# wenbowen123/BundleTrack

Hardware: AMD Instinct MI355X
Metric: Gauss-Newton iters/sec (K=15, 2k corr/frame-pair) + achieved HBM GB/s (higher is better)
Workload: dtype f32

## Files before the change

bundletrack_amd/csrc/btba_api.hip:

```cpp
#include <chrono>

#include "btba_host_common.hpp"
#include "btba_kernels.hpp"
#include "btba_solve_general.hpp"
#include "btba_chain.hpp"
#include "btba_solve_small.hpp"
#include "btba_solve_mid.hpp"

thread_local int btba_host::g_last_hip_error = 0;

extern "C" {

void btba_params_default(btba_params *p)
{
    if (!p) return;
    p->n_gn_iters = 7;
    p->n_pcg_iters = 5;
    p->robust_delta = 0.005f;
    p->dense_dist_thresh = 0.02f;
    p->dense_normal_thresh = (float)std::cos(45.0 / 180.0 * M_PI);
    p->depth_min = 0.1f;
    p->depth_max = 9999.0f;
    p->weight_sparse = 1.0f;
    p->weight_dense_depth = 1.0f;
// ... 541 lines not shown
        HIP_TRY(hipMemsetAsync(ws->dense_part.p, 0, sizeof(float) * (size_t)B * (Pd > 0 ? Pd : 1) * kDenseVals, ws->stream));
    }
    const bool compaction = use_zn && use_dense && (prm->flags & BTBA_FLAG_COMPACTION);
    const int chain_lay = zn_layout == 1 ? (compaction ? 3 : 1) : 0;
    const bool chain = chain_lay != 0 && !ws->chain_failed && ws->n_cus == 256 && ws->tune.chain > 0 && use_sparse && use_dense && !wsi && !wdi
                       && !trace && !atomic_sums && !a_global && !D.pre_assembled && N <= kChainMaxFrames && chunks <= kChainMaxParts && tiles <= kChainMaxParts
                       && !(prm->flags & (BTBA_FLAG_NO_FUSE | BTBA_FLAG_OVERLAP)) && !Z.frame_slot
                       && sizeof(float) * SolveLayout(N, D.n_dense_pairs, true, true).total <= kChainLdsBytes;
    const bool relayout = ws->tune.relayout && use_sparse && !corr24 && !pair_lens && !chain && prm->n_gn_iters >= 3 && !atomic_sums && !compaction
                          && (size_t)B * (size_t)corr_stride * sizeof(btba_entryj) >= ((size_t)4 << 20);
    if (relayout) { if ((rc = ws->corr24_tmp.ensure(sizeof(float2) * 192 * (((size_t)B * (size_t)corr_stride + 63) / 64)))) return rc; }
    const long long frames_bytes = use_dense ? (long long)B * N * npix * (use_zn ? 16 : 32) : 0;
    const long long corr_bytes = use_sparse ? (long long)B * (long long)corr_stride * (corr24 ? 24 : 32) : 0;
    const long long corr_per_instance = corr_bytes / B;
    int corr_nt_auto = B;
    if (use_dense && use_sparse && !compaction && frames_bytes + corr_bytes > ws->tune.last_level_cache)
        corr_nt_auto = (frames_bytes >= ws->tune.last_level_cache || corr_per_instance <= 0) ? 0 : (int)std::min<long long>(B, (ws->tune.last_level_cache - frames_bytes) / corr_per_instance);
    if (ws->tune.corr_nt_partial == 0 && corr_nt_auto < B) corr_nt_auto = 0;
    const int corr_nt_from = ws->tune.corr_nt >= 0 ? (ws->tune.corr_nt ? 0 : B) : corr_nt_auto;
    ChainDims Cn{};
    int plain_pairsum_in_lds = 0;
    auto pad32 = [](size_t floats) { return (floats + 31) & ~(size_t)31; };
    if (chain) {
        const int n_it = prm->n_gn_iters;
        D.pose_stride = (int)pad32(16 * (size_t)N); D.x_stride = (int)pad32(6 * (size_t)N);
        D.sp_stride = (unsigned)pad32((size_t)P * chunks * kSparseVals); D.dp_stride = (unsigned)pad32((size_t)Pd * tiles * kDenseVals);
        D.publish = 1;
        D.corr_nt_from = corr_nt_from;
        plain_pairsum_in_lds = D.pairsum_in_lds;
        D.pairsum_in_lds = 0;
        Cn.last_solve_external = 1;
        Cn.n_iter = n_it; Cn.n_inst = B; Cn.inst_per_xcd = (unsigned)((B + 7) / 8);
        Cn.items_d = (unsigned)tiles * (unsigned)D.n_dense_pairs; Cn.items_s = (unsigned)chunks * (unsigned)P;
        Cn.sparse_period = (unsigned)ws->tune.chain_sparse_period;
        if (Cn.sparse_period >= 2u && Cn.sparse_period * Cn.items_s > Cn.items_d + Cn.items_s) Cn.sparse_period = (Cn.items_d + Cn.items_s) / Cn.items_s;
        if (Cn.sparse_period < 2u) Cn.sparse_period = 0u;
        Cn.group = (Cn.sparse_period == 0u && ws->tune.chain_group > 1 && Cn.inst_per_xcd % (unsigned)ws->tune.chain_group == 0u && B % 8 == 0) ? (unsigned)ws->tune.chain_group : 1u;
        Cn.timeout_ticks = (long long)ws->tune.chain_timeout_ms * 100000ll;
        Cn.solve_prio = ws->tune.chain_solve_prio;
        Cn.debug_skip = ws->tune.chain_debug_skip;
        if (Cn.debug_skip & 16) D.publish = 0;
        Cn.pose_ring = (size_t)B * D.pose_stride; Cn.x_ring = (size_t)B * D.x_stride;
        Cn.sp_ring = (size_t)B * (size_t)D.sp_stride; Cn.dp_ring = (size_t)B * (size_t)D.dp_stride;
        Cn.ps_size = pad32((size_t)D.n_dense_pairs * kDenseVals); Cn.A_size = pad32((n + 2) * ld);
        if ((rc = ws->x.ensure(sizeof(float) * (n_it + 1) * Cn.x_ring))) return rc;
        if ((rc = ws->T.ensure(sizeof(float) * (n_it + 1) * Cn.pose_ring))) return rc;
        if ((rc = ws->Tinv.ensure(sizeof(float) * (n_it + 1) * Cn.pose_ring))) return rc;
        if ((rc = ws->sparse_part.ensure(sizeof(float) * n_it * Cn.sp_ring))) return rc;
        if ((rc = ws->dense_part.ensure(sizeof(float) * n_it * Cn.dp_ring))) return rc;
        if ((rc = ws->pairsum.ensure(sizeof(float) * (size_t)n_it * B * Cn.ps_size))) return rc;
        if ((rc = ws->big_A.ensure(sizeof(float) * (size_t)n_it * B * Cn.A_size))) return rc;
        const size_t sync_head = ((size_t)B * (n_it + 1) + 15) & ~(size_t)15;
        const size_t sync_ints = sync_head + (size_t)16 * B * (n_it + 1);
        if ((rc = ws->chain_sync.ensure(sizeof(int) * sync_ints))) return rc;
        if (!ws->chain_error) {
            HIP_TRY(hipHostMalloc(reinterpret_cast<void **>(&ws->chain_error), 64, hipHostMallocDefault));
            *ws->chain_error = 0;
        }
        HIP_TRY(hipMemsetAsync(ws->chain_sync.p, 0, sizeof(int) * sync_ints, ws->stream));
        Cn.flags = ws->chain_sync.as<int>(); Cn.arrivals = Cn.flags + B; Cn.published = Cn.flags + sync_head; Cn.error = ws->chain_error;
    }
    {
        const int total = B * N;
        if (chain) k_prepare_strided<<<(total + 63) / 64, 64, 0, ws->stream>>>(total, N, D.pose_stride, D.x_stride, poses, ws->x.as<float>(), ws->T.as<float>(), ws->Tinv.as<float>());
        else k_prepare<<<(total + 63) / 64, 64, 0, ws->stream>>>(total, poses, ws->x.as<float>(), ws->T.as<float>(), ws->Tinv.as<float>(), ws->tune.prepare_keep_T);
    }
    const uint32_t *lists_base = Z.lists;
    const int *counts_base = Z.counts;
    if (compaction && !lists_base) {
        if ((rc = ws->valid_lists.ensure(sizeof(uint32_t) * (size_t)B * N * npix))) return rc;
        if ((rc = ws->valid_counts.ensure(sizeof(int) * (size_t)B * N))) return rc;
        k_valid_lists<<<B * N, 1024, 0, ws->stream>>>(npix, reinterpret_cast<const float4 *>(Z.zn), ws->valid_lists.as<uint32_t>(), ws->valid_counts.as<int>(), nullptr);
        lists_base = ws->valid_lists.as<uint32_t>();
        counts_base = ws->valid_counts.as<int>();
    }
    if (Z.frame_slot && B != 1) return BTBA_EINVAL;
    D.frame_slot = Z.frame_slot;
    size_t blist_bytes = 0;
    if (!(zn_layout == 1 && use_dense && !compaction)) D.walk_blocks = 0;
    D.sparse_tail_256 = ws->tune.sparse_tail_256 >= 0 ? ws->tune.sparse_tail_256 : ((use_dense && !compaction) ? 256 : 0);
    if (D.walk_blocks) {
        const int bw = Wd / 8, bh = Hd / 8;
        const size_t band_blocks = (size_t)((bh + tiles - 1) / tiles) * bw;
        if (band_blocks > 1024) D.walk_blocks = 0;
        else {
            blist_bytes = 32 + sizeof(uint32_t) * band_blocks;
            if (ws->tune.block_skip) {
                if (Z.block_ranges) D.block_ranges = reinterpret_cast<const float2 *>(Z.block_ranges);
                else if (!Z.frame_slot) {
                    if ((rc = ws->block_ranges.ensure(sizeof(float2) * (size_t)B * N * bw * bh))) return rc;
                    k_block_ranges<<<dim3((unsigned)((bw * bh + kBlock / 64 - 1) / (kBlock / 64)), (unsigned)(B * N)), kBlock, 0, ws->stream>>>(Wd, Hd, reinterpret_cast<const float4 *>(Z.zn), nullptr, ws->block_ranges.as<float2>());
                    D.block_ranges = ws->block_ranges.as<float2>();
                }
            }
        }
    }
    int n_halves = (B >= 8 && (prm->flags & BTBA_FLAG_OVERLAP)) ? 2 : 1;
    if (n_halves == 2) n_halves = std::max(1, std::min({ ws->tune.overlap_groups, (int)btba_workspace::kMaxGroups, B / 2 }));
    for (int g = 1; g < n_halves; g++) {
        if (ws->aux_streams[g - 1]) continue;
        int prio_least = 0, prio_greatest = 0;
        HIP_TRY(hipDeviceGetStreamPriorityRange(&prio_least, &prio_greatest));
        HIP_TRY(hipStreamCreateWithPriority(&ws->aux_streams[g - 1], hipStreamNonBlocking, ws->tune.overlap_equal_prio ? 0 : prio_least));
        HIP_TRY(hipEventCreateWithFlags(&ws->ev_join[g - 1], hipEventDisableTiming));
        if (!ws->ev_fork) HIP_TRY(hipEventCreateWithFlags(&ws->ev_fork, hipEventDisableTiming));
    }
    struct Half { int b0, nb; hipStream_t st; } halves[btba_workspace::kMaxGroups];
    for (int g = 0; g < n_halves; g++) {
        const int lo = (int)((long long)B * g / n_halves), hi = (int)((long long)B * (g + 1) / n_halves);
        halves[g] = { lo, hi - lo, g == 0 ? ws->stream : ws->aux_streams[g - 1] };
    }
    if (n_halves > 1) {
        HIP_TRY(hipEventRecord(ws->ev_fork, ws->stream));
        for (int g = 1; g < n_halves; g++) HIP_TRY(hipStreamWaitEvent(ws->aux_streams[g - 1], ws->ev_fork, 0));
    }
    const size_t pairsum_floats = lds_pairs / sizeof(float);
    S.chain_iterations = 0;
    const size_t lut_bytes = sizeof(float) * (size_t)((Wd + Hd + 3) & ~3) + (zn_layout == 1 ? sizeof(float4) * (size_t)(Wd + Hd) : 0) + blist_bytes + (size_t)ws->tune.debug_lds_pad;
    if (chain) {
        const size_t chain_lds = std::max(lut_bytes, sizeof(float) * SolveLayout(N, D.n_dense_pairs, true, true).total);
        const unsigned per_inst = Cn.items_d + Cn.items_s + 1u;
        const unsigned grid = 8u * (unsigned)prm->n_gn_iters * Cn.inst_per_xcd * per_inst;
        if (!ws->tune.chain_trace_file.empty()) {
            const size_t trace_bytes = 32 * (size_t)grid + 64 * (size_t)prm->n_gn_iters * B;
            if ((rc = ws->chain_trace.ensure(trace_bytes))) return rc;
            HIP_TRY(hipMemsetAsync(ws->chain_trace.p, 0, trace_bytes, ws->stream));
            Cn.trace = ws->chain_trace.as<unsigned long long>();
            Cn.stamps = Cn.trace + 4 * (size_t)grid;
        }
        const float4 *corr_c = reinterpret_cast<const float4 *>(corr);
        size_t slot;
        if (Cn.debug_skip & 32) {
            ChainDims C1 = Cn;
            C1.n_iter = 1; C1.debug_skip |= 8; C1.trace = nullptr; C1.stamps = nullptr;
            const unsigned grid1 = 8u * Cn.inst_per_xcd * per_inst;
            if ((rc = ws->pairsum.ensure(sizeof(float) * (size_t)B * ((size_t)P * kSparseVals + (size_t)D.n_dense_pairs * kDenseVals + 64)))) return rc;
            for (int it = 0; it < prm->n_gn_iters; it++) {
                if ((rc = time_begin(ws, timing, 0, &slot))) return rc;
#define BTBA_CHAIN_ARGS1 D, C1, reinterpret_cast<const float4 *>(Z.zn), ws->T.as<float>(), ws->Tinv.as<float>(), ws->x.as<float>(), ws->dense_part.as<float>(), corr_c, pair_offsets, \
                        ws->sparse_part.as<float>(), compaction ? lists_base : nullptr, compaction ? counts_base : nullptr, ws->dense_pairs.as<int2>(), d_adj_off, d_adj, ws->solve_tab.as<int>(), \
                        ws->pairsum.as<float>(), ws->big_A.as<float>(), poses
                if (chain_lay == 1) k_chain<1><<<dim3(grid1), kBlock, chain_lds, ws->stream>>>(BTBA_CHAIN_ARGS1);
                else k_chain<3><<<dim3(grid1), kBlock, chain_lds, ws->stream>>>(BTBA_CHAIN_ARGS1);
#undef BTBA_CHAIN_ARGS1
                if ((rc = time_end(ws, slot))) return rc;
                if ((rc = time_begin(ws, timing, 2, &slot))) return rc;
                k_system_solve<false, false><<<B, kSolveBlock, lds_core, ws->stream>>>(D, it, ws->sparse_part.as<float>(), ws->dense_part.as<float>(), ws->dense_pairs.as<int2>(), d_adj_off, d_adj,
                    ws->x.as<float>(), ws->T.as<float>(), ws->Tinv.as<float>(), ws->pairsum.as<float>(), nullptr, nullptr, it == prm->n_gn_iters - 1 ? poses : nullptr, ws->solve_tab.as<int>());
                if ((rc = time_end(ws, slot))) return rc;
            }
            S.fused_sweeps = 1;
        } else {
        if ((rc = time_begin(ws, timing, 0, &slot))) return rc;
#define BTBA_CHAIN_ARGS D, Cn, reinterpret_cast<const float4 *>(Z.zn), ws->T.as<float>(), ws->Tinv.as<float>(), ws->x.as<float>(), ws->dense_part.as<float>(), corr_c, pair_offsets, \
                        ws->sparse_part.as<float>(), compaction ? lists_base : nullptr, compaction ? counts_base : nullptr, ws->dense_pairs.as<int2>(), d_adj_off, d_adj, ws->solve_tab.as<int>(), \
                        ws->pairsum.as<float>(), ws->big_A.as<float>(), poses
        if (chain_lay == 1) k_chain<1><<<dim3(grid), kBlock, chain_lds, ws->stream>>>(BTBA_CHAIN_ARGS);
        else k_chain<3><<<dim3(grid), kBlock, chain_lds, ws->stream>>>(BTBA_CHAIN_ARGS);
#undef BTBA_CHAIN_ARGS
        if ((rc = time_end(ws, slot))) return rc;
        if (Cn.last_solve_external) {
            const int il = prm->n_gn_iters - 1;
            SolveDims Dl = D;
            Dl.pairsum_in_lds = plain_pairsum_in_lds; Dl.publish = 0;
            if (!Dl.pairsum_in_lds) { if ((rc = ws->pairsum.ensure(std::max(sizeof(float) * (size_t)prm->n_gn_iters * B * Cn.ps_size, (size_t)B * lds_pairs + 16)))) return rc; }
            if ((rc = time_begin(ws, timing, 2, &slot))) return rc;
#define BTBA_LAST_SOLVE(LP) k_system_solve<LP, false><<<B, kSolveBlock, lds_bytes, ws->stream>>>(Dl, il, ws->sparse_part.as<float>() + il * Cn.sp_ring, ws->dense_part.as<float>() + il * Cn.dp_ring, \
                ws->dense_pairs.as<int2>(), d_adj_off, d_adj, ws->x.as<float>() + il * Cn.x_ring, ws->T.as<float>() + il * Cn.pose_ring, ws->Tinv.as<float>() + il * Cn.pose_ring, \
                ws->pairsum.as<float>(), nullptr, nullptr, poses, ws->solve_tab.as<int>())
// ... 798 lines not shown
```

bundletrack_amd/csrc/btba_kernels.hpp:

```cpp
#pragma once
#ifndef BTBA_FUSED_WAVES
#define BTBA_FUSED_WAVES 6
#endif
#if defined(BTBA_REFERENCE_ORDER) && !defined(BTBA_EXACT_DIV)
#define BTBA_EXACT_DIV 1
#endif
#include <type_traits>
#include <hip/hip_runtime.h>
#include <stdint.h>
#include "btba_device.hpp"

namespace btba {

constexpr int kBlock = 256;
constexpr int kSolveBlock = 1024;
constexpr int kSparseVals = 44;
constexpr int kDenseVals = 28;
constexpr float kEps = 0.000001f;
constexpr int kRedFloats = 4 * kSparseVals + 8;


struct SolveDims {
    int n_frames;
    int n_pairs;
    int n_dense_pairs;
    int npix, width, height;
    int sparse_chunks;
    int dense_tiles;
    int n_pcg;
    int use_sparse, use_dense;
    float fx, fy, cx, cy;
    float robust_delta, dist_thresh, normal_thresh, depth_min, depth_max;
    float dist2_thresh;
    float wm1, hm1, wm2, hm2;
    float w_sparse, w_dense;
    int64_t corr_stride;
    int trace_on;
    int64_t trace_record;
    int64_t tr_x, tr_T, tr_rhs, tr_prec, tr_pcg, tr_delta, tr_dpair, tr_A, tr_clk;
    int n_gn;
    int pairsum_in_lds;
    int pre_assembled;
    int walk_blocks;
    const int4 *dense_work;
    int work_formula;
    const float2 *block_ranges;
    int sparse_tail_256;
    int tile_major;
    int *order_flag;
    int atomic_sums;
    int corr24;
    int64_t corr_entry0;
    const uint32_t *pair_lens;
    float zn_ki[16];
    float zn_scale_w, zn_scale_h;
    int zn_simple;
    const int *frame_slot;
    int pose_stride, x_stride;
    unsigned sp_stride, dp_stride;
    float2 *corr24_out;
    unsigned long long *live_blocks;
    int publish;
    int corr_nt_from;
};

__device__ __forceinline__ size_t frame_slot_of(const SolveDims &D, size_t f) { return D.frame_slot ? (size_t)D.frame_slot[f] : f; }

__device__ __forceinline__ int pair_index(int i, int j, int n) { return i * n - i * (i + 1) / 2 + (j - i - 1); }

__device__ __forceinline__ Mat4 load_mat4(const float *p)
{
    Mat4 m;
    const float4 *q = reinterpret_cast<const float4 *>(p);
    float4 a = q[0], b = q[1], c = q[2], d = q[3];
    m.m[0] = a.x; m.m[1] = a.y; m.m[2] = a.z; m.m[3] = a.w;
    m.m[4] = b.x; m.m[5] = b.y; m.m[6] = b.z; m.m[7] = b.w;
    m.m[8] = c.x; m.m[9] = c.y; m.m[10] = c.z; m.m[11] = c.w;
    m.m[12] = d.x; m.m[13] = d.y; m.m[14] = d.z; m.m[15] = d.w;
    return m;
}
__device__ __forceinline__ Mat4 load_mat4_uniform(const float *p)
{
    Mat4 m;
    const float4 a = ld_const_f4(p), b = ld_const_f4(p + 4), c = ld_const_f4(p + 8), d = ld_const_f4(p + 12);
    m.m[0] = a.x; m.m[1] = a.y; m.m[2] = a.z; m.m[3] = a.w;
    m.m[4] = b.x; m.m[5] = b.y; m.m[6] = b.z; m.m[7] = b.w;
    m.m[8] = c.x; m.m[9] = c.y; m.m[10] = c.z; m.m[11] = c.w;
    m.m[12] = d.x; m.m[13] = d.y; m.m[14] = d.z; m.m[15] = d.w;
    return m;
}
__device__ __forceinline__ void store_mat4(float *p, const Mat4 &m)
{
    float4 *q = reinterpret_cast<float4 *>(p);
// ... 642 lines not shown
    const unsigned pb = (unsigned)b * (unsigned)D.pose_stride;
    dense_stage_M(red, T + pb + 16 * fi);
    DenseCtx C;
    C.Tij = mat_mul(load_mat4(Tinv + pb + 16 * fi), load_mat4(T + pb + 16 * fj));
#pragma unroll
    for (int e = 0; e < 12; e++) C.Tij.m[e] = __builtin_bit_cast(float, __builtin_amdgcn_readfirstlane(__builtin_bit_cast(int, C.Tij.m[e])));
    C.cam_t = nullptr; C.nrm_t = nullptr;
    C.fx = D.fx; C.fy = D.fy; C.cx = D.cx; C.cy = D.cy; C.depth_min = D.depth_min; C.depth_max = D.depth_max;
    C.normal_thresh = D.normal_thresh; C.dist2_thresh = D.dist_thresh * D.dist_thresh;
    C.delta = D.robust_delta; C.delta2 = D.robust_delta * D.robust_delta; C.w_dense = D.w_dense;
    C.W = D.width; C.H = D.height;
    const size_t slot_t = (size_t)__builtin_amdgcn_readfirstlane((int)frame_slot_of(D, fb + fi));
    const size_t slot_s = (size_t)__builtin_amdgcn_readfirstlane((int)frame_slot_of(D, fb + fj));
    const float4 *zn_t = zn + slot_t * (size_t)D.npix, *zn_s = zn + slot_s * (size_t)D.npix;
    const int n_src = LISTS ? valid_counts[slot_s] : D.npix;
    const uint32_t *list = LISTS ? valid_lists + slot_s * (size_t)D.npix : nullptr;
    const int per = (n_src + D.dense_tiles - 1) / D.dense_tiles;
    const int lo = min(n_src, per * tile), hi = min(n_src, per * (tile + 1));
    const float inv_w = 1.0f / (float)D.width;
    float acc[kDenseVals];
#pragma unroll
    for (int k = 0; k < kDenseVals; k++) acc[k] = 0.0f;

    int t = lo + (int)threadIdx.x;
    int s_n = (t < hi) ? (LISTS ? (int)list[t] : t) : 0;
    int px_i = s_n % D.width, py_i = s_n / D.width;
    const int step_x = kBlock % D.width, step_y = kBlock / D.width;
    float4 zs_n = make_float4(0.f, 0.f, 0.f, 0.f);
    if (t < hi) zs_n = zn_s[s_n];
    for (; t < hi; t += kBlock) {
        const float4 zs = zs_n;
        const int s = s_n;
        if (t + kBlock < hi) { s_n = LISTS ? (int)list[t + kBlock] : t + kBlock; zs_n = zn_s[s_n]; }
        int px, py;
        if (!LISTS) {
            px = px_i; py = py_i;
            px_i += step_x; py_i += step_y;
            if (px_i >= D.width) { px_i -= D.width; py_i++; }
        } else {
            py = (int)((float)s * inv_w);
            py -= (py * D.width > s) ? 1 : 0;
            py += ((py + 1) * D.width <= s) ? 1 : 0;
            px = s - py * D.width;
        }
        const float3 cp = zn_backproject<SIMPLE>(D.zn_ki, lut_x[px], lut_y[py], zs.x);
        const PixelGeom g = pixel_geom(C, make_float4(cp.x, cp.y, cp.z, 1.0f), make_float4(zs.y, zs.z, zs.w, 0.0f));
        if (__builtin_amdgcn_ballot_w64(g.valid) == 0ull) continue;
        const char *zt = reinterpret_cast<const char *>(zn_t);
        const float4 z00 = *reinterpret_cast<const float4 *>(zt + ((unsigned)g.i00 << 4)), z10 = *reinterpret_cast<const float4 *>(zt + ((unsigned)g.i10 << 4));
        const float4 z01 = *reinterpret_cast<const float4 *>(zt + ((unsigned)g.i01 << 4)), z11 = *reinterpret_cast<const float4 *>(zt + ((unsigned)g.i11 << 4));
        const float xia = lut_x[g.xa], xib = lut_x[g.xb], yia = lut_y[g.ya], yib = lut_y[g.yb];
        const float3 c00 = zn_backproject<SIMPLE>(D.zn_ki, xia, yia, z00.x), c10 = zn_backproject<SIMPLE>(D.zn_ki, xib, yia, z10.x);
        const float3 c01 = zn_backproject<SIMPLE>(D.zn_ki, xia, yib, z01.x), c11 = zn_backproject<SIMPLE>(D.zn_ki, xib, yib, z11.x);
        pixel_accumulate(C, g, make_float4(c00.x, c00.y, c00.z, 1.f), make_float4(c10.x, c10.y, c10.z, 1.f), make_float4(c01.x, c01.y, c01.z, 1.f), make_float4(c11.x, c11.y, c11.z, 1.f),
                         make_float4(z00.y, z00.z, z00.w, 0.f), make_float4(z10.y, z10.z, z10.w, 0.f), make_float4(z01.y, z01.z, z01.w, 0.f), make_float4(z11.y, z11.z, z11.w, 0.f), acc);
    }
    float *out = partials + ((unsigned)b * D.dp_stride + (unsigned)(D.atomic_sums ? p : p * D.dense_tiles + tile) * (unsigned)kDenseVals);
    dense_epilogue(acc, red, out, D.atomic_sums ? 1 : D.publish ? 2 : 0);
}

struct PinholeCtx {
    float R[9], t[3];
    float fx, fy, cx, cy, wm1, hm1, wm2, hm2, w16, normal_thresh, dist2_thresh, wdelta, w_dense, ybase4;
    unsigned row16;
    unsigned zmin_bits, zrange_bits;
};

template <int IMM> __device__ __forceinline__ float4 gather16_imm(const char *base, unsigned byte_off) { return *reinterpret_cast<const float4 *>(base + (size_t)byte_off + IMM); }
__device__ __forceinline__ unsigned lds_address(const void *p) { return (unsigned)(unsigned long)(const __attribute__((address_space(3))) char *)p; }
__device__ __forceinline__ float2 lds_f32x2_abs(unsigned addr) { const __attribute__((address_space(3))) float *q = (const __attribute__((address_space(3))) float *)(unsigned long)addr; return make_float2(q[0], q[1]); }
__device__ __forceinline__ float min_raw(float a, float b) { float r; asm("v_min_f32 %0, %1, %2" : "=v"(r) : "v"(a), "v"(b)); return r; }
__device__ __forceinline__ float fma_nd(float a, float b, float c) { float d; asm("v_fma_f32 %0, %1, %2, %3" : "=&v"(d) : "v"(a), "v"(b), "v"(c)); return d; }
__device__ __forceinline__ float min_raw_s(float a, float bound) { float r; asm("v_min_f32 %0, %2, %1" : "=v"(r) : "v"(a), "s"(bound)); return r; }
__device__ __forceinline__ float clamp0_s(float a, float bound) { float r; asm("v_med3_f32 %0, %1, %2, 0" : "=v"(r) : "v"(a), "s"(bound)); return r; }
__device__ __forceinline__ float sgpr(float x) { return __builtin_bit_cast(float, __builtin_amdgcn_readfirstlane(__builtin_bit_cast(int, x))); }

__device__ __forceinline__ float pinhole_lut_entry(const SolveDims &D, int e)
{
    const bool is_x = e < D.width;
    const float c = (float)(is_x ? zn_src_coord(e, D.zn_scale_w) : zn_src_coord(e - D.width, D.zn_scale_h));
    return is_x ? D.zn_ki[0] * c + D.zn_ki[2] : D.zn_ki[5] * c + D.zn_ki[6];
}

__device__ __forceinline__ bool block_is_live(const SolveDims &D, const float (&R)[9], const float (&t)[3], float2 zr, int bxl, int byg)
{
    zr.x = fmaxf(zr.x, D.depth_min); zr.y = fminf(zr.y, D.depth_max);
    bool live = zr.x <= zr.y;
    if (live) {
        const float xa = pinhole_lut_entry(D, 8 * bxl), xb = pinhole_lut_entry(D, 8 * bxl + 7);
        const float ya = pinhole_lut_entry(D, D.width + 8 * byg), yb = pinhole_lut_entry(D, D.width + 8 * byg + 7);
        float ulo = INFINITY, uhi = -INFINITY, vlo = INFINITY, vhi = -INFINITY, zq = INFINITY;
#pragma unroll
        for (int k = 0; k < 4; k++) {
            const float x = (k & 1) ? xb : xa, y = (k & 2) ? yb : ya;
            const float rx = R[0] * x + R[1] * y + R[2], ry = R[3] * x + R[4] * y + R[5], rz = R[6] * x + R[7] * y + R[8];
#pragma unroll
            for (int e = 0; e < 2; e++) {
                const float d = e ? zr.y : zr.x;
                const float qx = rx * d + t[0], qy = ry * d + t[1], qz = rz * d + t[2];
                const float rq = fast_rcp(qz);
                const float u = qx * D.fx * rq + D.cx, v = qy * D.fy * rq + D.cy;
                ulo = fminf(ulo, u); uhi = fmaxf(uhi, u); vlo = fminf(vlo, v); vhi = fmaxf(vhi, v); zq = fminf(zq, qz);
            }
        }
        const float m = 0.01f;
        const bool outside = (uhi < -0.5f - m) | (ulo > (float)D.width - 0.5f + m) | (vhi < -0.5f - m) | (vlo > (float)D.height - 0.5f + m);
        live = !(zq > 1e-3f && outside);
    }
    return live;
}

__device__ __forceinline__ bool block_is_live_planes(const SolveDims &D, const float4 *colA, const float4 *rowB, const float (&t)[3], float2 zr, int bxl, int byg)
{
    zr.x = fmaxf(zr.x, D.depth_min); zr.y = fminf(zr.y, D.depth_max);
    bool live = zr.x <= zr.y;
    if (live) {
        const float4 ca = colA[8 * bxl], cb = colA[8 * bxl + 7], ra = rowB[8 * byg], rb = rowB[8 * byg + 7];
        const float m = 0.01f;
        const float cL = D.cx + 0.5f + m, cR = D.cx - ((float)D.width - 0.5f + m), cT = D.cy + 0.5f + m, cB = D.cy - ((float)D.height - 0.5f + m);
        float maxL = -INFINITY, minR = INFINITY, maxT = -INFINITY, minB = INFINITY, zq = INFINITY;
#pragma unroll
        for (int k = 0; k < 4; k++) {
            const float4 cx4 = (k & 1) ? cb : ca, ry4 = (k & 2) ? rb : ra;
            const float rx = cx4.x + ry4.x, ry = cx4.y + ry4.y, rz = cx4.z + ry4.z;
            const float fxrx = rx * D.fx, fyry = ry * D.fy;
            const float aL = fxrx + cL * rz, aR = fxrx + cR * rz, aT = fyry + cT * rz, aB = fyry + cB * rz;
            maxL = fmaxf(maxL, fmaxf(aL * zr.x, aL * zr.y)); minR = fminf(minR, fminf(aR * zr.x, aR * zr.y));
            maxT = fmaxf(maxT, fmaxf(aT * zr.x, aT * zr.y)); minB = fminf(minB, fminf(aB * zr.x, aB * zr.y));
            zq = fminf(zq, fminf(rz * zr.x, rz * zr.y));
        }
        const float bL = D.fx * t[0] + cL * t[2], bR = D.fx * t[0] + cR * t[2], bT = D.fy * t[1] + cT * t[2], bB = D.fy * t[1] + cB * t[2];
        const bool outside = (maxL + bL < 0.0f) | (minR + bR > 0.0f) | (maxT + bT < 0.0f) | (minB + bB > 0.0f);
        live = !((zq + t[2] > 1e-3f) && outside);
    }
    return live;
}

__device__ __forceinline__ void dense_work_item(const SolveDims &D, int q, int &fi, int &fj, int &p)
{
    if (D.work_formula) {
        int d = 1, rem = q;
        while (rem >= D.n_frames - d) { rem -= D.n_frames - d; d++; }
        p = pair_index(rem, rem + d, D.n_frames);
        fi = D.work_formula == 1 ? rem : rem + d;
        fj = D.work_formula == 1 ? rem + d : rem;
    } else {
        const int4 w = ld_const_i4(D.dense_work + q);
        fi = w.x; fj = w.y; p = w.z;
    }
}

template <int WALK>
__device__ __forceinline__ void dense_block_pinhole(const SolveDims &D, const float4 *__restrict__ zn, int q,
                                                    const float *__restrict__ T, const float *__restrict__ Tinv,
                                                    float *__restrict__ partials, int tile, int b, float *red,
                                                    const uint32_t *__restrict__ valid_lists, const int *__restrict__ valid_counts, float *lut)
{
    const unsigned tid = item_tid();
    int fi, fj, p;
    dense_work_item(D, q, fi, fj, p);
    const size_t fb = (size_t)b * D.n_frames;
    const size_t slot_t = (size_t)__builtin_amdgcn_readfirstlane((int)frame_slot_of(D, fb + fi));
    const size_t slot_s = (size_t)__builtin_amdgcn_readfirstlane((int)frame_slot_of(D, fb + fj));
    const unsigned pb = (unsigned)b * (unsigned)D.pose_stride;
    const Mat4 Tinv_i = load_mat4_uniform(Tinv + pb + 16 * fi), T_j = load_mat4_uniform(T + pb + 16 * fj);
    float m_stage = 0.0f;
    if (tid >= 64 && tid < 64 + 36) {
        const float *T_target = T + pb + 16 * fi;
        const int e = (int)tid - 64, r = e / 6, c = e % 6;
        if (r < 3) m_stage = (c < 3) ? T_target[4 * r + c] : 0.0f;
        else {
            const int qq = r - 3, qa = (qq + 1) % 3, qb = (qq + 2) % 3;
            m_stage = (c < 3) ? T_target[4 * qa + 3] * T_target[4 * qb + c] - T_target[4 * qb + 3] * T_target[4 * qa + c] : T_target[4 * qq + (c - 3)];
        }
    }
    const int bw = D.width >> 3, bh = D.height >> 3;
    const int rows_per = (bh + D.dense_tiles - 1) / D.dense_tiles;
    const int r0 = min(bh, rows_per * tile), r1 = min(bh, rows_per * (tile + 1));
    const int nb = (WALK == 2) ? (r1 - r0) * bw : 0;
    const float2 *rng = (WALK == 2 && D.block_ranges) ? D.block_ranges + slot_s * (size_t)(bw * bh) + (size_t)r0 * bw : nullptr;
    const float2 zr0 = (rng && (int)tid < nb) ? rng[tid] : make_float2(0.0f, 0.0f);
    const float2 zr1 = (rng && (int)tid + kBlock < nb) ? rng[tid + kBlock] : make_float2(0.0f, 0.0f);
    const Mat4 Tij = mat_mul(Tinv_i, T_j);
    PinholeCtx C;
#pragma unroll
    for (int r = 0; r < 3; r++) {
#pragma unroll
        for (int c = 0; c < 3; c++) C.R[3 * r + c] = sgpr(Tij.m[4 * r + c]);
        C.t[r] = sgpr(Tij.m[4 * r + 3]);
    }
    float4 *colA = reinterpret_cast<float4 *>(lut + ((D.width + D.height + 3) & ~3));
    float4 *rowB = colA + D.width;
    for (int e = (int)tid; e < D.width + D.height; e += kBlock) {
        const float l = pinhole_lut_entry(D, e);
        lut[e] = l;
        if (e < D.width) colA[e] = make_float4(C.R[0] * l, C.R[3] * l, C.R[6] * l, 0.0f);
        else rowB[e - D.width] = make_float4(C.R[1] * l + C.R[2], C.R[4] * l + C.R[5], C.R[7] * l + C.R[8], 0.0f);
    }
    if (tid >= 64 && tid < 64 + 36) red[4 * kDenseVals + kDenseVals + 4 + ((int)tid - 64)] = m_stage;
    int *hdr = reinterpret_cast<int *>(rowB + D.height);
    unsigned *blist = reinterpret_cast<unsigned *>(hdr + 8);
    int n_live = 0;
    if (WALK == 2) {
        __syncthreads();
        const int lane_c = (int)tid & 63, wave_c = __builtin_amdgcn_readfirstlane((int)tid >> 6);
        for (int c0 = 0; c0 < nb; c0 += 2 * kBlock) {
            const int idx0 = c0 + (int)tid, idx1 = idx0 + kBlock;
            bool live0 = false, live1 = false;
            unsigned code0 = 0, code1 = 0;
            if (idx0 < nb) {
                const int byl = idx0 / bw, bxl = idx0 - byl * bw, byg = r0 + byl;
                code0 = ((unsigned)byg << 16) | (unsigned)bxl;
                live0 = rng ? block_is_live_planes(D, colA, rowB, C.t, c0 ? rng[idx0] : zr0, bxl, byg) : true;
            }
            if (idx1 < nb) {
                const int byl = idx1 / bw, bxl = idx1 - byl * bw, byg = r0 + byl;
                code1 = ((unsigned)byg << 16) | (unsigned)bxl;
                live1 = rng ? block_is_live_planes(D, colA, rowB, C.t, c0 ? rng[idx1] : zr1, bxl, byg) : true;
            }
            const unsigned long long bal0 = __builtin_amdgcn_ballot_w64(live0), bal1 = __builtin_amdgcn_ballot_w64(live1);
            if (lane_c == 0) { hdr[wave_c] = __popcll(bal0); hdr[4 + wave_c] = __popcll(bal1); }
            __syncthreads();
            int base0 = n_live, total0 = 0, base1 = 0, total1 = 0;
#pragma unroll
            for (int w = 0; w < kBlock / 64; w++) {
                const int t0 = hdr[w], t1 = hdr[4 + w];
                if (w < wave_c) { base0 += t0; base1 += t1; }
                total0 += t0; total1 += t1;
            }
            base1 += n_live + total0;
            const int before0 = __builtin_amdgcn_mbcnt_hi((unsigned)(bal0 >> 32), __builtin_amdgcn_mbcnt_lo((unsigned)bal0, 0));
            const int before1 = __builtin_amdgcn_mbcnt_hi((unsigned)(bal1 >> 32), __builtin_amdgcn_mbcnt_lo((unsigned)bal1, 0));
            if (live0) blist[base0 + before0] = code0;
            if (live1) blist[base1 + before1] = code1;
            n_live += total0 + total1;
            __syncthreads();
        }
    } else __syncthreads();
    C.fx = D.fx; C.fy = D.fy; C.cx = D.cx; C.cy = D.cy;
    C.wm1 = D.wm1; C.hm1 = D.hm1; C.wm2 = D.wm2; C.hm2 = D.hm2;
    C.w16 = 16.0f * (float)D.width; C.row16 = 16u * (unsigned)D.width;
    C.ybase4 = 4.0f * (float)D.width;
    C.normal_thresh = D.normal_thresh; C.dist2_thresh = D.dist2_thresh;
    C.wdelta = D.w_dense * D.robust_delta; C.w_dense = D.w_dense;
    C.zmin_bits = __float_as_uint(D.depth_min) + 1u; C.zrange_bits = __float_as_uint(D.depth_max) - __float_as_uint(D.depth_min) - 1u;
    const float4 *zn_t = zn + slot_t * (size_t)D.npix, *zn_s = zn + slot_s * (size_t)D.npix;
    constexpr bool LISTS = (WALK == 1);
    float acc[kDenseVals];
#pragma unroll
    for (int k = 0; k < kDenseVals; k++) acc[k] = 0.0f;
    int n_ok = 0;

    const char *tap_row0 = reinterpret_cast<const char *>(zn_t), *tap_row1 = tap_row0 + C.row16;
    const float lut_addr_f = (float)lds_address(lut), ybase4_abs = C.ybase4 + lut_addr_f;
    auto pixel = [&](const float4 &zs, unsigned ox, unsigned oy) {
        const float d = zs.x;
        const bool src_ok = (__float_as_uint(d) - C.zmin_bits) < C.zrange_bits;
        const float4 ra = *reinterpret_cast<const float4 *>(reinterpret_cast<const char *>(colA) + ox), rb = *reinterpret_cast<const float4 *>(reinterpret_cast<const char *>(colA) + oy);
        const float qx = (ra.x + rb.x) * d + C.t[0], qy = (ra.y + rb.y) * d + C.t[1], qz = (ra.z + rb.z) * d + C.t[2];
        const float rqz = fast_rcp(qz);
        const float u = qx * C.fx * rqz + C.cx, v = qy * C.fy * rqz + C.cy;
        const float uc = clamp0_s(u, C.wm1), vc = clamp0_s(v, C.hm1);
        const bool valid = src_ok & (fabsf(u - uc) < 0.5f) & (fabsf(v - vc) < 0.5f);
        const unsigned long long valid_mask = __builtin_amdgcn_ballot_w64(src_ok) & __builtin_amdgcn_ballot_w64(fabsf(u - uc) < 0.5f) & __builtin_amdgcn_ballot_w64(fabsf(v - vc) < 0.5f);
        if (valid_mask == 0ull) return;
        const float nqx = C.R[0] * zs.y + C.R[1] * zs.z + C.R[2] * zs.w;
        const float nqy = C.R[3] * zs.y + C.R[4] * zs.z + C.R[5] * zs.w;
        const float nqz = C.R[6] * zs.y + C.R[7] * zs.z + C.R[8] * zs.w;
        const float fx0 = min_raw_s(floorf(uc), C.wm2), fy0 = min_raw_s(floorf(vc), C.hm2);
        const float alpha = uc - fx0, beta = vc - fy0;
        const unsigned o00 = (unsigned)(fy0 * C.w16 + 16.0f * fx0);
        float4 z00, z10, z01, z11;
#pragma clang diagnostic push
#pragma clang diagnostic ignored "-Wconditional-uninitialized"
        if (valid) { z00 = gather16_imm<0>(tap_row0, o00); z10 = gather16_imm<16>(tap_row0, o00); z01 = gather16_imm<0>(tap_row1, o00); z11 = gather16_imm<16>(tap_row1, o00); }
#pragma clang diagnostic pop
        const float2 xi2 = lds_f32x2_abs((unsigned)(4.0f * fx0 + lut_addr_f)), yi2 = lds_f32x2_abs((unsigned)(4.0f * fy0 + ybase4_abs));
        const float a0 = 1.0f - alpha, b0 = 1.0f - beta;
        const float c00 = b0 * a0, c10 = b0 * alpha, c01 = beta * a0, c11 = beta * alpha;
        const float t10 = c10 * z10.x, t01 = c01 * z01.x, t11 = c11 * z11.x;
        const float s0x = fma_nd(c00, z00.x, t01), s0y = fma_nd(c00, z00.x, t10);
        const float s1x = fma_nd(c10, z10.x, t11), s1y = fma_nd(c01, z01.x, t11);
        const float cix = fma_nd(xi2.x, s0x, xi2.y * s1x);
        const float ciy = fma_nd(yi2.x, s0y, yi2.y * s1y);
        const float ciz = s0x + s1x;
        const float nix = fma_nd(c11, z11.y, fma_nd(c01, z01.y, fma_nd(c00, z00.y, c10 * z10.y)));
        const float niy = fma_nd(c11, z11.z, fma_nd(c01, z01.z, fma_nd(c00, z00.z, c10 * z10.z)));
        const float niz = fma_nd(c11, z11.w, fma_nd(c01, z01.w, fma_nd(c00, z00.w, c10 * z10.w)));
        const float dx = qx - cix, dy = qy - ciy, dz = qz - ciz;
        const float dist2 = fma_nd(dz, dz, fma_nd(dx, dx, dy * dy));
        const float dn = fma_nd(nqz, niz, fma_nd(nqx, nix, nqy * niy));
        const unsigned long long ok_mask = valid_mask & __builtin_amdgcn_ballot_w64((__float_as_uint(ciz) - C.zmin_bits) < C.zrange_bits)
                                         & __builtin_amdgcn_ballot_w64(dn >= C.normal_thresh) & __builtin_amdgcn_ballot_w64(dist2 <= C.dist2_thresh);
        n_ok += __popcll(ok_mask);
        if (__builtin_amdgcn_inverse_ballot_w64(ok_mask)) {
            const float res = fma_nd(dz, niz, fma_nd(dx, nix, dy * niy));
            const float wgt = min_raw_s(C.wdelta * fast_rsq(res * res), C.w_dense);
            const float a[6] = { nix, niy, niz, niy * qz - niz * qy, niz * qx - nix * qz, nix * qy - niy * qx };
            int k = 0;
            typedef float f2v __attribute__((ext_vector_type(2)));
            f2v pr[6];
// ... 180 lines not shown
```

Baseline: 217,500.

## Precompute separable per-column/row hull bounds for block liveness culling

Replaces the per-block liveness test, which evaluated four corners from LUT planes, with a separable form. Per-column and per-row hull extrema (left/right/top/bottom and min z) are precomputed once into LDS by the last wave, so each block test becomes sums of two entries scaled by its depth range. It also replaces the integer division used to get the block row with a float reciprocal multiply. The cost is extra LDS workspace and a different bound: max(a)+max(b) is looser than the max over corners, so fewer blocks may be culled. The float-based division also adds a precision assumption.

After: 220,100 (median of 6 runs). 1.01x the previous value.

```diff
diff --git a/bundletrack_amd/csrc/btba_api.hip b/bundletrack_amd/csrc/btba_api.hip
--- a/bundletrack_amd/csrc/btba_api.hip
+++ b/bundletrack_amd/csrc/btba_api.hip
@@ -647,9 +647,9 @@
     if (D.walk_blocks) {
         const int bw = Wd / 8, bh = Hd / 8;
         const size_t band_blocks = (size_t)((bh + tiles - 1) / tiles) * bw;
-        if (band_blocks > 1024) D.walk_blocks = 0;
+        if (band_blocks > (size_t)kMaxBandBlocks) D.walk_blocks = 0;
         else {
-            blist_bytes = 32 + sizeof(uint32_t) * band_blocks;
+            blist_bytes = 32 * (size_t)(bw + bh) + 32 + sizeof(uint32_t) * band_blocks;
             if (ws->tune.block_skip) {
                 if (Z.block_ranges) D.block_ranges = reinterpret_cast<const float2 *>(Z.block_ranges);
                 else if (!Z.frame_slot) {
diff --git a/bundletrack_amd/csrc/btba_hull.hpp b/bundletrack_amd/csrc/btba_hull.hpp
--- /dev/null
+++ b/bundletrack_amd/csrc/btba_hull.hpp
@@ -0,0 +1,78 @@
+#pragma once
+#include <cmath>
+
+#if defined(__HIPCC__)
+#define BTBA_HULL_FN __host__ __device__ inline
+#elif defined(__GNUC__) && !defined(__clang__)
+#define BTBA_HULL_FN __attribute__((optimize("fp-contract=off"))) inline
+#else
+#define BTBA_HULL_FN inline
+#endif
+#if defined(__clang__)
+#define BTBA_HULL_NO_CONTRACT _Pragma("clang fp contract(off)")
+#else
+#define BTBA_HULL_NO_CONTRACT
+#endif
+
+namespace btba_hull {
+
+constexpr float kMargin = 0.01f;
+
+struct HullForms { float fx, fy, cL, cR, cT, cB; };
+
+BTBA_HULL_FN HullForms hull_forms(float fx, float fy, float cx, float cy, int width, int height)
+{
+    BTBA_HULL_NO_CONTRACT
+    HullForms F;
+    F.fx = fx; F.fy = fy;
+    F.cL = cx + 0.5f + kMargin; F.cR = cx - ((float)width - 0.5f + kMargin);
+    F.cT = cy + 0.5f + kMargin; F.cB = cy - ((float)height - 0.5f + kMargin);
+    return F;
+}
+
+struct HullEntry { float lmax, rmin, tmax, bmin, zmin; };
+
+BTBA_HULL_FN HullEntry hull_entry(const float (&R)[9], const HullForms &F, bool row, float la, float lb)
+{
+    BTBA_HULL_NO_CONTRACT
+    const float mx = row ? R[1] : R[0], my = row ? R[4] : R[3], mz = row ? R[7] : R[6];
+    const float ox = row ? R[2] : 0.0f, oy = row ? R[5] : 0.0f, oz = row ? R[8] : 0.0f;
+    const float ax = mx * la + ox, ay = my * la + oy, az = mz * la + oz;
+    const float bx = mx * lb + ox, by = my * lb + oy, bz = mz * lb + oz;
+    const float fa = F.fx * ax, fb = F.fx * bx, ga = F.fy * ay, gb = F.fy * by;
+    const float La = fa + F.cL * az, Lb = fb + F.cL * bz, Ra = fa + F.cR * az, Rb = fb + F.cR * bz;
+    const float Ta = ga + F.cT * az, Tb = gb + F.cT * bz, Ba = ga + F.cB * az, Bb = gb + F.cB * bz;
+    const float poison = 0.0f * (((La + Lb) + (Ra + Rb)) + ((Ta + Tb) + (Ba + Bb)));
+    HullEntry e;
+    e.lmax = fmaxf(La, Lb) + poison; e.rmin = fminf(Ra, Rb) + poison;
+    e.tmax = fmaxf(Ta, Tb) + poison; e.bmin = fminf(Ba, Bb) + poison;
+    e.zmin = fminf(az, bz) + poison;
+    return e;
+}
+
+struct HullBias { float bL, bR, bT, bB, tz; };
+
+BTBA_HULL_FN HullBias hull_bias(const HullForms &F, const float (&t)[3])
+{
+    BTBA_HULL_NO_CONTRACT
+    HullBias b;
+    b.bL = F.fx * t[0] + F.cL * t[2]; b.bR = F.fx * t[0] + F.cR * t[2];
+    b.bT = F.fy * t[1] + F.cT * t[2]; b.bB = F.fy * t[1] + F.cB * t[2];
+    b.tz = t[2] + 0.0f * (t[0] + t[1]);
+    return b;
+}
+
+BTBA_HULL_FN bool hull_block_live(const HullEntry &c, const HullEntry &r, const HullBias &b, float zlo, float zhi, float depth_min, float depth_max)
+{
+    BTBA_HULL_NO_CONTRACT
+    zlo = fmaxf(zlo, depth_min); zhi = fminf(zhi, depth_max);
+    if (!(zlo <= zhi)) return false;
+    const float L = c.lmax + r.lmax, Rr = c.rmin + r.rmin, T = c.tmax + r.tmax, B = c.bmin + r.bmin, Z = c.zmin + r.zmin;
+    const float maxL = fmaxf(L * zlo, L * zhi), minR = fminf(Rr * zlo, Rr * zhi);
+    const float maxT = fmaxf(T * zlo, T * zhi), minB = fminf(B * zlo, B * zhi);
+    const float zq = fminf(Z * zlo, Z * zhi);
+    const bool outside = (maxL + b.bL < 0.0f) | (minR + b.bR > 0.0f) | (maxT + b.bT < 0.0f) | (minB + b.bB > 0.0f);
+    return !((zq + b.tz > 1e-3f) && outside);
+}
+
+}
diff --git a/bundletrack_amd/csrc/btba_kernels.hpp b/bundletrack_amd/csrc/btba_kernels.hpp
--- a/bundletrack_amd/csrc/btba_kernels.hpp
+++ b/bundletrack_amd/csrc/btba_kernels.hpp
@@ -9,6 +9,7 @@
 #include <hip/hip_runtime.h>
 #include <stdint.h>
 #include "btba_device.hpp"
+#include "btba_hull.hpp"
 
 namespace btba {
 
@@ -817,59 +818,8 @@
     return is_x ? D.zn_ki[0] * c + D.zn_ki[2] : D.zn_ki[5] * c + D.zn_ki[6];
 }
 
-__device__ __forceinline__ bool block_is_live(const SolveDims &D, const float (&R)[9], const float (&t)[3], float2 zr, int bxl, int byg)
-{
-    zr.x = fmaxf(zr.x, D.depth_min); zr.y = fminf(zr.y, D.depth_max);
-    bool live = zr.x <= zr.y;
-    if (live) {
-        const float xa = pinhole_lut_entry(D, 8 * bxl), xb = pinhole_lut_entry(D, 8 * bxl + 7);
-        const float ya = pinhole_lut_entry(D, D.width + 8 * byg), yb = pinhole_lut_entry(D, D.width + 8 * byg + 7);
-        float ulo = INFINITY, uhi = -INFINITY, vlo = INFINITY, vhi = -INFINITY, zq = INFINITY;
-#pragma unroll
-        for (int k = 0; k < 4; k++) {
-            const float x = (k & 1) ? xb : xa, y = (k & 2) ? yb : ya;
-            const float rx = R[0] * x + R[1] * y + R[2], ry = R[3] * x + R[4] * y + R[5], rz = R[6] * x + R[7] * y + R[8];
-#pragma unroll
-            for (int e = 0; e < 2; e++) {
-                const float d = e ? zr.y : zr.x;
-                const float qx = rx * d + t[0], qy = ry * d + t[1], qz = rz * d + t[2];
-                const float rq = fast_rcp(qz);
-                const float u = qx * D.fx * rq + D.cx, v = qy * D.fy * rq + D.cy;
-                ulo = fminf(ulo, u); uhi = fmaxf(uhi, u); vlo = fminf(vlo, v); vhi = fmaxf(vhi, v); zq = fminf(zq, qz);
-            }
-        }
-        const float m = 0.01f;
-        const bool outside = (uhi < -0.5f - m) | (ulo > (float)D.width - 0.5f + m) | (vhi < -0.5f - m) | (vlo > (float)D.height - 0.5f + m);
-        live = !(zq > 1e-3f && outside);
-    }
-    return live;
-}
-
-__device__ __forceinline__ bool block_is_live_planes(const SolveDims &D, const float4 *colA, const float4 *rowB, const float (&t)[3], float2 zr, int bxl, int byg)
-{
-    zr.x = fmaxf(zr.x, D.depth_min); zr.y = fminf(zr.y, D.depth_max);
-    bool live = zr.x <= zr.y;
-    if (live) {
-        const float4 ca = colA[8 * bxl], cb = colA[8 * bxl + 7], ra = rowB[8 * byg], rb = rowB[8 * byg + 7];
-        const float m = 0.01f;
-        const float cL = D.cx + 0.5f + m, cR = D.cx - ((float)D.width - 0.5f + m), cT = D.cy + 0.5f + m, cB = D.cy - ((float)D.height - 0.5f + m);
-        float maxL = -INFINITY, minR = INFINITY, maxT = -INFINITY, minB = INFINITY, zq = INFINITY;
-#pragma unroll
-        for (int k = 0; k < 4; k++) {
-            const float4 cx4 = (k & 1) ? cb : ca, ry4 = (k & 2) ? rb : ra;
-            const float rx = cx4.x + ry4.x, ry = cx4.y + ry4.y, rz = cx4.z + ry4.z;
-            const float fxrx = rx * D.fx, fyry = ry * D.fy;
-            const float aL = fxrx + cL * rz, aR = fxrx + cR * rz, aT = fyry + cT * rz, aB = fyry + cB * rz;
-            maxL = fmaxf(maxL, fmaxf(aL * zr.x, aL * zr.y)); minR = fminf(minR, fminf(aR * zr.x, aR * zr.y));
-            maxT = fmaxf(maxT, fmaxf(aT * zr.x, aT * zr.y)); minB = fminf(minB, fminf(aB * zr.x, aB * zr.y));
-            zq = fminf(zq, fminf(rz * zr.x, rz * zr.y));
-        }
-        const float bL = D.fx * t[0] + cL * t[2], bR = D.fx * t[0] + cR * t[2], bT = D.fy * t[1] + cT * t[2], bB = D.fy * t[1] + cB * t[2];
-        const bool outside = (maxL + bL < 0.0f) | (minR + bR > 0.0f) | (maxT + bT < 0.0f) | (minB + bB > 0.0f);
-        live = !((zq + t[2] > 1e-3f) && outside);
-    }
-    return live;
-}
+constexpr int kMaxBandBlocks = 1024;
+
 
 __device__ __forceinline__ void dense_work_item(const SolveDims &D, int q, int &fi, int &fj, int &p)
 {
@@ -916,6 +866,7 @@
     const float2 *rng = (WALK == 2 && D.block_ranges) ? D.block_ranges + slot_s * (size_t)(bw * bh) + (size_t)r0 * bw : nullptr;
     const float2 zr0 = (rng && (int)tid < nb) ? rng[tid] : make_float2(0.0f, 0.0f);
     const float2 zr1 = (rng && (int)tid + kBlock < nb) ? rng[tid + kBlock] : make_float2(0.0f, 0.0f);
+    const int lane_c = (int)tid & 63, wave_c = __builtin_amdgcn_readfirstlane((int)tid >> 6);
     const Mat4 Tij = mat_mul(Tinv_i, T_j);
     PinholeCtx C;
 #pragma unroll
@@ -933,25 +884,46 @@
         else rowB[e - D.width] = make_float4(C.R[1] * l + C.R[2], C.R[4] * l + C.R[5], C.R[7] * l + C.R[8], 0.0f);
     }
     if (tid >= 64 && tid < 64 + 36) red[4 * kDenseVals + kDenseVals + 4 + ((int)tid - 64)] = m_stage;
-    int *hdr = reinterpret_cast<int *>(rowB + D.height);
+    float *hull = reinterpret_cast<float *>(rowB + D.height);
+    const int n_ent = bw + bh;
+    int *hdr = reinterpret_cast<int *>(hull + 8 * n_ent);
     unsigned *blist = reinterpret_cast<unsigned *>(hdr + 8);
     int n_live = 0;
     if (WALK == 2) {
+        namespace H = btba_hull;
+        const H::HullForms F = H::hull_forms(D.fx, D.fy, D.cx, D.cy, D.width, D.height);
+        const H::HullBias hb = H::hull_bias(F, C.t);
+        if (rng) {
+#pragma clang loop vectorize(disable) interleave(disable) unroll(disable)
+            for (int e = (int)tid - (kBlock - 64); e >= 0 && e < n_ent; e += 64) {
+                const bool row = e >= bw;
+                const int px = row ? D.width + 8 * (e - bw) : 8 * e;
+                const H::HullEntry h = H::hull_entry(C.R, F, row, pinhole_lut_entry(D, px), pinhole_lut_entry(D, px + 7));
+                *reinterpret_cast<float4 *>(hull + 8 * e) = make_float4(h.lmax, h.rmin, h.tmax, h.bmin);
+                hull[8 * e + 4] = h.zmin;
+            }
+        }
         __syncthreads();
-        const int lane_c = (int)tid & 63, wave_c = __builtin_amdgcn_readfirstlane((int)tid >> 6);
+        const float inv_bw = fast_rcp((float)bw);
+        auto is_live = [&](const float2 &zr, int bxl, int byg) {
+            const float *ce = hull + 8 * bxl, *re = hull + 8 * (bw + byg);
+            const float4 c4 = *reinterpret_cast<const float4 *>(ce), r4 = *reinterpret_cast<const float4 *>(re);
+            const H::HullEntry hc = { c4.x, c4.y, c4.z, c4.w, ce[4] }, hr = { r4.x, r4.y, r4.z, r4.w, re[4] };
+            return H::hull_block_live(hc, hr, hb, zr.x, zr.y, D.depth_min, D.depth_max);
+        };
         for (int c0 = 0; c0 < nb; c0 += 2 * kBlock) {
             const int idx0 = c0 + (int)tid, idx1 = idx0 + kBlock;
             bool live0 = false, live1 = false;
             unsigned code0 = 0, code1 = 0;
             if (idx0 < nb) {
-                const int byl = idx0 / bw, bxl = idx0 - byl * bw, byg = r0 + byl;
+                const int byl = (int)(((float)idx0 + 0.5f) * inv_bw), bxl = idx0 - byl * bw, byg = r0 + byl;
                 code0 = ((unsigned)byg << 16) | (unsigned)bxl;
-                live0 = rng ? block_is_live_planes(D, colA, rowB, C.t, c0 ? rng[idx0] : zr0, bxl, byg) : true;
+                live0 = rng ? is_live(c0 ? rng[idx0] : zr0, bxl, byg) : true;
             }
             if (idx1 < nb) {
-                const int byl = idx1 / bw, bxl = idx1 - byl * bw, byg = r0 + byl;
+                const int byl = (int)(((float)idx1 + 0.5f) * inv_bw), bxl = idx1 - byl * bw, byg = r0 + byl;
                 code1 = ((unsigned)byg << 16) | (unsigned)bxl;
-                live1 = rng ? block_is_live_planes(D, colA, rowB, C.t, c0 ? rng[idx1] : zr1, bxl, byg) : true;
+                live1 = rng ? is_live(c0 ? rng[idx1] : zr1, bxl, byg) : true;
             }
             const unsigned long long bal0 = __builtin_amdgcn_ballot_w64(live0), bal1 = __builtin_amdgcn_ballot_w64(live1);
             if (lane_c == 0) { hdr[wave_c] = __popcll(bal0); hdr[4 + wave_c] = __popcll(bal1); }
```
